# Wil-Lee/NN_BVH

Measured on AMD Instinct MI355X. Metric: Mray/s (closest-hit + any-hit), higher is better.
Workload: dtype f32; 1 GPU; crown, 1000x1400: one wavefront pass of 8 spp per step (8 spp per GPU-film) — primary, bounce-1 and bounce-2 closest-hit, shadow any-hit towards the light quads (batches pre-generated, hence independent: ONE launch; the dependent form is dependent_step), rays in --ray-order tile (a caller-side order the reference's integrator does not form: ray_order_probe), RecordShadowRayResult + RGBFilm::AddSam; sample_sets=4, geometry=procedural stand-in for crown (3548192 tris; data/crown.npz absent), tree=sah, triangles=3548192, nodes=7032259, rays_primary=11200000, rays_bounce=7410327, rays_bounce2=4392209, parallelism=tile-sharded x1, BVH replicated, film all-gather after the pass

## Files before the change

### nn_bvh_amd/build.py

```python
import concurrent.futures
import hashlib
import os
import shutil
import subprocess

HERE = os.path.dirname(os.path.abspath(__file__))
CSRC = os.path.join(HERE, "csrc")
LIB = os.path.join(HERE, "libnnbvh_hip.so")
SOURCES = ["bvh_trace.hip", "wavefront.hip", "wavefront2.hip", "wavefront_items.hip", "bvh_build_gpu.hip", "bvh_bake.hip", "interaction.hip", "film.hip", "kd_trace.hip", "kd_build_gpu.hip", "kd_bake.hip", "bvh_capi.cpp", "capi_two_level.cpp", "capi_trace.cpp", "capi_kd.cpp", "capi_wavefront.cpp", "capi_shading.cpp", "bvh_build.cpp", "kd_build.cpp"]
HEADERS = ["bvh_trace.h", "trace_instance.h", "top_table.h", "trace_math.h", "stream_access.h", "spawn_math.h", "anim_math.h", "alpha_texture_math.h", "wavefront2.h", "walk_math.h", "wavefront.h", "bvh_build_gpu.h", "interaction.h", "interaction_math.h", "wavefront_items.h", "kd_trace.h", "kd_build_gpu.h", "kd_device_util.h", "nnbvh_internal.h", "capi_internal.h", os.path.join("..", "..", "include", "nnbvh.h")]
CFLAGS = ["-O3", "--offload-arch=gfx950", "-ffp-contract=off", "-fPIC", "-std=c++17",
          "-Wall", "-Wno-unused-function", "-Wno-pass-failed"]
FLAGS = CFLAGS + ["-shared"]


def _hipcc():
    hipcc = shutil.which("hipcc") or "/opt/rocm/bin/hipcc"
    if not os.path.exists(hipcc):
        raise RuntimeError("hipcc not found: cannot build libnnbvh_hip.so")
    return hipcc


def _sources():
    return [s for s in SOURCES if os.path.exists(os.path.join(CSRC, s))]


def _deps_mtime():
    deps = [os.path.join(CSRC, f) for f in HEADERS] + [os.path.abspath(__file__)]
    return max(os.path.getmtime(d) for d in deps if os.path.exists(d))


def _stale():
    if not os.path.exists(LIB):
        return True
    t = os.path.getmtime(LIB)
    return _deps_mtime() > t or any(os.path.getmtime(os.path.join(CSRC, s)) > t for s in _sources())


def _build(out, extra=(), force=False, verbose=False, jobs=None):
    hipcc = _hipcc()
    tag = hashlib.sha1(" ".join(extra).encode()).hexdigest()[:10] if extra else "product"
    objdir = os.path.join(HERE, "_obj", tag)
    os.makedirs(objdir, exist_ok=True)
    hdr_t = _deps_mtime()
    todo, objs = [], []
    for s in _sources():
        src = os.path.join(CSRC, s)
        obj = os.path.join(objdir, s.rsplit(".", 1)[0] + ".o")
        objs.append(obj)
        if force or not os.path.exists(obj) or os.path.getmtime(obj) < max(hdr_t, os.path.getmtime(src)):
            todo.append([hipcc] + CFLAGS + list(extra) + ["-c", "-o", obj, src])

    def run(cmd):
        if verbose:
            print(" ".join(cmd), flush=True)
        subprocess.run(cmd, check=True, cwd=CSRC)

    jobs = jobs or min(len(todo) or 1, max(1, (os.cpu_count() or 2) - 1), 6)
    with concurrent.futures.ThreadPoolExecutor(jobs) as ex:
        list(ex.map(run, todo))
    run([hipcc, "--offload-arch=gfx950", "-shared", "-fPIC", "-o", out] + objs)
    return out


def build_stats(verbose=False):
    return _build(os.path.join(HERE, "libnnbvh_hip_stats.so"), ["-DNNBVH_STATS"], verbose=verbose)


def build_variant(name, defines, verbose=False, flags=()):
    return _build(os.path.join(HERE, f"libnnbvh_hip_{name}.so"), list(flags) + [f"-D{d}" for d in defines],
                  verbose=verbose)


def build(force=False, verbose=False):
    if not force and not _stale():
        return LIB
    return _build(LIB, force=force, verbose=verbose)


if __name__ == "__main__":
    import sys
    if len(sys.argv) > 1:
        print(build_variant(sys.argv[1], sys.argv[2:], verbose=True))
    else:
        print(build(force=True, verbose=True))
```

### nn_bvh_amd/csrc/bvh_capi.cpp

```cpp
#include <algorithm>
#include <cmath>
#include <cstring>
#include <limits>
#include <vector>

#include "alpha_texture_math.h"
#include "bvh_build_gpu.h"
#include "capi_internal.h"
#include "top_table.h"

namespace nnbvh {

static thread_local std::string g_error;
void set_error(const std::string &msg) { g_error = msg; }

}

using namespace nnbvh;

static bool validate_tree(const nnbvh_linear_node *nodes, int root, int n_tree, const nnbvh_prim *prims,
                          int n_prims, bool allow_instances, std::vector<uint8_t> &covered,
                          std::vector<uint8_t> &leaf_last, int *depth_out) {
    if (n_tree < 1) {
        set_error("scene_create: tree has no nodes");
        return false;
    }
    const int n_nodes = root + n_tree;
    struct Frame {
        int node, end, depth;
    };
    std::vector<Frame> st;
    st.push_back({root, n_nodes, 0});
    int visited = 0, max_depth = 0;
    while (!st.empty()) {
        Frame f = st.back();
        st.pop_back();
        ++visited;
        if (f.node < 0 || f.node >= f.end) {
            set_error("scene_create: node index outside its subtree range");
            return false;
        }
        max_depth = std::max(max_depth, f.depth);
        const nnbvh_linear_node &nd = nodes[f.node];
        for (int k = 0; k < 3; ++k)
            if (!(nd.pmin[k] <= nd.pmax[k])) {
                set_error("scene_create: node bounds with min > max (or NaN)");
                return false;
            }
        if (nd.nprims > 0) {
            if (f.node + 1 != f.end) {
                set_error("scene_create: leaf does not close its subtree range (not a DFS layout)");
                return false;
            }
            if (nd.offset < 0 || (int64_t)nd.offset + nd.nprims > n_prims) {
                set_error("scene_create: leaf primitive range out of bounds");
                return false;
            }
            for (int i = 0; i < nd.nprims; ++i) {
                if (covered[(size_t)nd.offset + i]) {
                    set_error("scene_create: primitive referenced by two leaves");
                    return false;
                }
                covered[(size_t)nd.offset + i] = 1;
                if (!allow_instances && prims[(size_t)nd.offset + i].kind == NNBVH_PRIM_INSTANCE) {
                    set_error("scene_create: nested instances are not supported");
                    return false;
                }
            }
            leaf_last[(size_t)nd.offset + nd.nprims - 1] = 1;
        } else {
            if (nd.axis > 2) {
                set_error("scene_create: interior node axis > 2");
                return false;
            }
            const int c0 = f.node + 1, c1 = nd.offset;
            if (c1 <= c0 || c1 >= f.end) {
                set_error("scene_create: secondChildOffset outside the node's subtree range");
                return false;
            }
            st.push_back({c1, f.end, f.depth + 1});
            st.push_back({c0, c1, f.depth + 1});
        }
    }
    if (visited != n_tree) {
        set_error("scene_create: unreachable nodes in the array");
        return false;
    }
    *depth_out = max_depth;
    return true;
}

// ... 683 lines not shown
    }
    std::memcpy(out, s->bounds, sizeof s->bounds);
    return NNBVH_OK;
}

int nnbvh_scene_info(const nnbvh_scene *s, int64_t out[6]) {
    if (!s || !out) {
        set_error("scene_info: null argument");
        return NNBVH_ERR_ARG;
    }
    out[0] = s->n_interior;
    out[1] = s->n_slots;
    out[2] = s->depth;
    out[3] = (int64_t)s->device_bytes;
    out[4] = grid_blocks(const_cast<nnbvh_scene *>(s), 0);
    out[5] = s->window;
    return NNBVH_OK;
}

int nnbvh_scene_read(const nnbvh_scene *s, int what, void *out, size_t bytes) {
    if (!s || !out) {
        set_error("scene_read: null argument");
        return NNBVH_ERR_ARG;
    }
    if (what < 0 || what > 4) {
        set_error("scene_read: unknown array (0 interior records, 1 primitive stream, 2 animation table, 3 alpha-texture "
                  "table, 4 alpha texel pool)");
        return NNBVH_ERR_ARG;
    }
    if (what >= 3) {
        if (!s->d_alpha_tex) {
            set_error("scene_read: the scene has no alpha textures");
            return NNBVH_ERR_ARG;
        }
        const void *from = what == 3 ? (const void *)s->d_alpha_tex : (const void *)s->d_alpha_texels;
        const size_t size = what == 3 ? (size_t)s->n_alpha_tex * 48 : (size_t)s->n_alpha_texels * 4;
        if (bytes != size) {
            set_error("scene_read: " + std::to_string(bytes) + " bytes asked for, the array has " + std::to_string(size));
            return NNBVH_ERR_ARG;
        }
        DeviceGuard guard(s->device);
        if (!guard.ok) return NNBVH_ERR_DEVICE;
        if (!hip_ok(hipDeviceSynchronize(), "scene_read") || !hip_ok(hipMemcpy(out, from, bytes, hipMemcpyDeviceToHost), "scene_read"))
            return NNBVH_ERR_DEVICE;
        return NNBVH_OK;
    }
    if (what == 2 && !s->d_anim) {
        set_error("scene_read: the scene has no animation table");
        return NNBVH_ERR_ARG;
    }
    const void *src = what == 0 ? (const void *)s->d_wide : what == 1 ? (const void *)s->d_prims : (const void *)s->d_anim;
    const size_t have = what == 0   ? (size_t)s->n_interior * sizeof(WideNode)
                        : what == 1 ? (size_t)s->n_slots * 16
                                    : (size_t)s->n_anim * kAnimStride * sizeof(float);
    if (bytes != have) {
        set_error("scene_read: " + std::to_string(bytes) + " bytes asked for, the array has " + std::to_string(have));
        return NNBVH_ERR_ARG;
    }
    if (bytes == 0) return NNBVH_OK;
    DeviceGuard guard(s->device);
    if (!guard.ok) return NNBVH_ERR_DEVICE;
    if (!hip_ok(hipDeviceSynchronize(), "scene_read") || !hip_ok(hipMemcpy(out, src, bytes, hipMemcpyDeviceToHost), "scene_read"))
        return NNBVH_ERR_DEVICE;
    return NNBVH_OK;
}

int nnbvh_scene_sched_stats(nnbvh_scene *s, uint64_t out[20], int reset) {
    if (!s || !out) {
        set_error("scene_sched_stats: null argument");
        return NNBVH_ERR_ARG;
    }
    std::memset(out, 0, nnbvh::kSchedStatWords * sizeof(uint64_t));
    if (!s->d_stats) return NNBVH_OK;
    DeviceGuard guard(s->device);
    if (!guard.ok) return NNBVH_ERR_DEVICE;
    if (!hip_ok(hipDeviceSynchronize(), "scene_sched_stats") ||
        !hip_ok(hipMemcpy(out, s->d_stats, nnbvh::kSchedStatWords * sizeof(uint64_t), hipMemcpyDeviceToHost),
                "scene_sched_stats"))
        return NNBVH_ERR_DEVICE;
    if (reset) (void)hipMemset(s->d_stats, 0, nnbvh::kSchedStatWords * sizeof(unsigned long long));
    return NNBVH_OK;
}

int nnbvh_scene_set_option(nnbvh_scene *s, const char *key, int value) {
    if (!s || !key) {
        set_error("set_option: null argument");
        return NNBVH_ERR_ARG;
    }
    std::lock_guard<std::mutex> lock(s->mu);
    std::string k(key);
    if (k == "stack_window") {
        if (value != 4 && value != 8 && value != 16) {
            set_error("set_option: stack_window must be 4, 8 or 16");
            return NNBVH_ERR_ARG;
        }
        s->window = value;
    } else if (k == "blocks_per_cu") {
        if (value < 0 || value > 8) {
            set_error("set_option: blocks_per_cu must be 0..8");
            return NNBVH_ERR_ARG;
        }
        s->blocks_per_cu = value;
    } else if (k == "int_repeat") {
        if (value < 1 || value > 16) {
            set_error("set_option: int_repeat must be 1..16");
            return NNBVH_ERR_ARG;
        }
        s->int_repeat = value;
    } else if (k == "host_chunk") {
        if (value < 1024) {
            set_error("set_option: host_chunk must be at least 1024 rays");
            return NNBVH_ERR_ARG;
        }
        s->host_chunk = value;
    } else if (k == "prim_repeat") {
        if (value < 1 || value > 16) {
            set_error("set_option: prim_repeat must be 1..16");
            return NNBVH_ERR_ARG;
        }
        s->prim_repeat = value;
    } else if (k == "fused_batches") {
        s->fused_batches = value ? 1 : 0;
    } else if (k == "top_table") {
        s->use_top = value ? 1 : 0;
    } else if (k == "top_burst") {
        if (value < 1 || value > 65) {
            set_error("set_option: top_burst must be 1..65");
            return NNBVH_ERR_ARG;
        }
        s->top_burst = value;
    } else if (k == "xcd_queues") {
        s->xcd_queues = value ? 1 : 0;
    } else if (k == "prim_weight") {
        if (value < 1 || value > 64) {
            set_error("set_option: prim_weight must be 1..64");
            return NNBVH_ERR_ARG;
        }
        s->prim_weight = value;
    } else if (k == "refill_weight") {
        if (value < 1 || value > 64) {
            set_error("set_option: refill_weight must be 1..64");
            return NNBVH_ERR_ARG;
        }
        s->refill_weight = value;
    } else {
        set_error("set_option: unknown key");
        return NNBVH_ERR_ARG;
    }
    return NNBVH_OK;
}

}

Workspace *nnbvh::workspace_for(nnbvh_scene *s, hipStream_t stream) {
    auto it = s->workspaces.find(stream);
    if (it != s->workspaces.end()) return &it->second;
    Workspace w;
    const size_t spill_bytes = (size_t)std::max(s->depth - 2, 1) * (size_t)s->max_grid_threads * sizeof(uint2);
    if (!hip_ok(hipMalloc((void **)&w.queue, kMaxFusedBatches * kMaxQueues * kQueueStrideWords * sizeof(unsigned)),
                "hipMalloc(queue)"))
        return nullptr;
    if (!hip_ok(hipMalloc((void **)&w.spill, spill_bytes), "hipMalloc(spill)")) {
        (void)hipFree(w.queue);
        return nullptr;
    }
    return &(s->workspaces[stream] = w);
// ... 2 lines not shown
```

### nn_bvh_amd/csrc/bvh_trace.h

```cpp
#pragma once
#include <hip/hip_runtime.h>
#include <stdint.h>

#include "../../include/nnbvh.h"
#include "nnbvh_internal.h"
#include "trace_instance.h"
#include "walk_math.h"

namespace nnbvh {

constexpr int kBlockThreads = 256;
constexpr int kMaxQueues = 8;
constexpr int kQueueStrideWords = 32;
constexpr int kMaxFusedBatches = 4;
constexpr int kSchedStatWords = 20;
constexpr int kFusedIndexBits = 28;

struct TraceParams {
    const float4 *wide;
    const float4 *prims;
    float rootMin[3], rootMax[3];
    int rootRef;
    const nnbvh_ray *rays;
    nnbvh_hit *hits;
    uint8_t *occluded;
    int32_t *visitedOut;
    int32_t *testsOut;
    long n;
    const int32_t *nDev;
    unsigned *queue;
    int nQueues;
    int primWeight;
    int refillWeight;
    int hasHostPrims;
    int intRepeat;
    int primRepeat;
    int fits32;
    unsigned long long *stats;
    uint2 *spill;
    const float *anim;
    int nBatches;
    unsigned anyMask;
    const nnbvh_ray *bRays[kMaxFusedBatches];
    void *bOut[kMaxFusedBatches];
    long bN[kMaxFusedBatches];
    const int32_t *bNDev[kMaxFusedBatches];
    nnbvh_ray_soa soa;
    nnbvh_ray_soa bSoa[kMaxFusedBatches];
    int hcCap;
    int32_t *hcCount;
    int32_t *hcBefore;
    int32_t *hcPrim;
    int32_t *hcInst;
    int bHcCap[kMaxFusedBatches];
    int32_t *bHcCount[kMaxFusedBatches];
    int32_t *bHcBefore[kMaxFusedBatches];
    int32_t *bHcPrim[kMaxFusedBatches];
    int32_t *bHcInst[kMaxFusedBatches];
    ShadingMeshDevice wMesh;
    WalkParams walk;
    const float4 *alphaTex;
    const float *alphaTexels;
    const float4 *top;
    int nTop;
    int topBurst;
};

hipError_t launch_zero_queue(unsigned *queue, int words, hipStream_t stream);
hipError_t launch_zero_words(int32_t *words, long n, int maxBlocks, hipStream_t stream);

hipError_t launch_trace(const TraceInstance &is, const TraceParams &p, int blocks, hipStream_t stream, int *occupancy);

}
```

### nn_bvh_amd/csrc/bvh_trace.hip

```cpp
#include <hip/hip_runtime.h>
#include <stdint.h>
#include <array>
#include <cstring>
#include <utility>

#include "bvh_trace.h"
#include "alpha_texture_math.h"
#include "anim_math.h"
#include "spawn_math.h"
#include "stream_access.h"
#include "trace_math.h"
#include "walk_math.h"

namespace nnbvh {

constexpr int kDone = (int)0x80000000;
constexpr int kReturn = (int)0x80000001;
constexpr int kEnter = (int)0x80000002;

#ifndef NNBVH_MINW_CLOSEST
#define NNBVH_MINW_CLOSEST 6
#endif
#ifndef NNBVH_MINW_ANY
#define NNBVH_MINW_ANY 6
#endif
#ifndef NNBVH_LEAN_EXTRA_WAVES
#define NNBVH_LEAN_EXTRA_WAVES 2
#endif
#ifndef NNBVH_MINW_ALPHA
#define NNBVH_MINW_ALPHA 5
#endif
#ifndef NNBVH_MINW_ALPHA_PATCH
#define NNBVH_MINW_ALPHA_PATCH 3
#endif
#ifndef NNBVH_MINW_ALPHA_TEX
#define NNBVH_MINW_ALPHA_TEX 4
#endif
#ifndef NNBVH_MINW_WALK_LEAN
#define NNBVH_MINW_WALK_LEAN 4
#endif
#ifndef NNBVH_MINW_WALK
#define NNBVH_MINW_WALK 4
#endif
constexpr int min_waves(int modew, int inst, int patch, int alpha) {
    if (inst) return 1;
    if (modew >= 4) return patch ? NNBVH_MINW_WALK : NNBVH_MINW_WALK_LEAN;
    if (alpha == 2) return NNBVH_MINW_ALPHA_PATCH;
    if (alpha == 3) return NNBVH_MINW_ALPHA_TEX;
    if (alpha) return NNBVH_MINW_ALPHA;
    return ((modew == 0 || modew == 3) ? NNBVH_MINW_CLOSEST : NNBVH_MINW_ANY) + (patch ? 0 : NNBVH_LEAN_EXTRA_WAVES);
}
#ifndef NNBVH_ANIM_ENTER_WEIGHT
#define NNBVH_ANIM_ENTER_WEIGHT 8
#endif
template <typename T>
__device__ __forceinline__ T pick_batch(const T (&a)[kMaxFusedBatches], int b) {
    static_assert(kMaxFusedBatches == 4, "written out for four batches");
    return b == 0 ? a[0] : (b == 1 ? a[1] : (b == 2 ? a[2] : a[3]));
}

#define BVH_BEGIN_RAY(R0, R1)                                                                                         \
    do {                                                                                                              \
        r.o = {(R0).x, (R0).y, (R0).z};                                                                               \
        tMax = (R0).w;                                                                                                \
        const V3 d = {(R1).x, (R1).y, (R1).z};                                                                        \
        if (PATCH) {                                                                                                  \
            cold[kColdD][lane] = d.x;                                                                                 \
            cold[kColdD + 1][lane] = d.y;                                                                             \
            cold[kColdD + 2][lane] = d.z;                                                                             \
        }                                                                                                             \
                                                                                          \
        r.inv = {1.0f / d.x, 1.0f / d.y, 1.0f / d.z};                                                                 \
        ray_shear(r, d);                                                                                              \
        if constexpr (kTop) {                                                                                         \
            hit0 = __int_as_float(-1);                                                                                \
            hit1 = hit2 = hit3 = 0.0f;                                                                                \
        } else if (MODE == 0 || MODE == 3) {                                                                          \
            cold[kColdHit][lane] = __int_as_float(-1);                                                                \
            cold[kColdHit + 1][lane] = 0.0f;                                                                          \
            cold[kColdHit + 2][lane] = 0.0f;                                                                          \
            cold[kColdHit + 3][lane] = 0.0f;                                                                          \
        }                                                                                                             \
        if (INST) {                                                                                                   \
            cold[kHitInst][lane] = 0.0f;                                                                              \
            cold[kCurInst][lane] = 0.0f;                                                                              \
            cold[kColdTime][lane] = (R1).w;                                 \
            floor = -1;                                                                                               \
        }                                                                                                             \
        if (!kLean && (HOSTC || p.hasHostPrims)) cold[kColdHost][lane] = 0.0f;           \
        if constexpr (WALK != 0) {                                                                                    \
            cold[kWalkD][lane] = (R1).x;                                                                              \
            cold[kWalkD + 1][lane] = (R1).y;                                                                          \
            cold[kWalkD + 2][lane] = (R1).z;                                                                          \
            cold[kWalkTime][lane] = (R1).w;                                                                           \
            cold[kWalkTMax][lane] = (R0).w;                                                                           \
        }                                                                                                             \
        visited = 1;                                                                                    \
        tests = 0;                                                                                                    \
        found = false;                                                                                                \
        sp = base = 0;                                                                                                \
        float tEntry;                                                                                                 \
        const bool rootHit = slab_partial(p.rootMin[0], p.rootMin[1], p.rootMin[2], p.rootMax[0], p.rootMax[1],       \
                                          p.rootMax[2], r, tEntry) &&                                                 \
                             (tEntry < tMax);                                                                         \
        cur = rootHit ? p.rootRef : kDone;                                                                            \
    } while (0)

template <int MODEW, int W, int INST, int PATCH, int ALPHA = 0, int SOA = 0, int HOSTC = 0>
__global__ __launch_bounds__(kBlockThreads, min_waves(MODEW, INST, PATCH, ALPHA))
void trace_kernel(TraceParams p) {
    constexpr int WALK = MODEW >= 4 ? MODEW - 3 : 0;
    constexpr int MODE = WALK ? 0 : MODEW;
    static_assert(!WALK || (MODEW <= 5 && W == 8 && INST != 2 && !ALPHA && !SOA && !HOSTC),
                  "walk instances: the plain record-reading closest-hit form at window 8");
    static_assert(PATCH || !INST, "two-level scenes need the ray direction");
    static_assert(PATCH || !ALPHA, "the alpha test hashes the ray direction");
    static_assert(ALPHA != 3 || (INST == 0 && W == 8 && MODE != 3), "textured alpha: flat scenes, window 8, modes 0 / 1 / 2");
    static_assert(!HOSTC || (PATCH && (MODE == 0 || MODE == 2 || (MODE == 3 && !ALPHA && W == 8)) && !SOA),
                  "candidate mode: general instances of modes 0 / 2 / 3");
    __shared__ float s_stack[kBlockThreads / 64][W][2][64];
    constexpr bool kLean = !PATCH && !INST;
    constexpr int kColdRi = 0, kColdD = 1, kColdHit = kLean ? 0 : (PATCH ? 4 : 1),
                  kColdHost = kColdHit + ((MODE == 0 || MODE == 3) ? 4 : 0);
    constexpr int kColdBase = kColdHost + (kLean ? 0 : 1);
    constexpr int kSaveO = kColdBase, kSaveInv = kColdBase + 3, kSaveShear = kColdBase + 6,
                  kSaveKz = kColdBase + 9, kSaveTmax = kColdBase + 10, kSaveD = kColdBase + 11,
                  kResume = kColdBase + 14, kCurInst = kColdBase + 15, kHitInst = kColdBase + 16,
                  kInnerHit = kColdBase + 17, kColdTime = kColdBase + 18, kPendSlot = kColdBase + 19;
    constexpr int kColdWalk = kColdBase + (INST ? 20 : 0);
    [[maybe_unused]] constexpr int kWalkD = kColdWalk, kWalkTime = kColdWalk + 3, kWalkTMax = kColdWalk + 4,
                                   kWalkCalls = kColdWalk + 5;
    constexpr int kColdFields = kColdWalk + (WALK ? 6 : 0);
    constexpr bool kTop = kLean && MODEW == 3;

    const int lane = threadIdx.x & 63;
    const int wave = threadIdx.x >> 6;
    const int gtid = blockIdx.x * kBlockThreads + threadIdx.x;
    float(*stk)[2][64] = s_stack[wave];
    float(*cold)[64] = nullptr;
    [[maybe_unused]] const float4 *top = nullptr;
    if constexpr (kTop) {
        __shared__ float4 s_top[kTopRecords * 4];
        static_assert(kTopRecords * 4 <= kBlockThreads, "one float4 per thread copies the table");
        if ((int)threadIdx.x < p.nTop * 4) s_top[threadIdx.x] = p.top[threadIdx.x];
        __syncthreads();
        top = s_top;
    } else {
        __shared__ float s_cold[kBlockThreads / 64][kColdFields > 0 ? kColdFields : 1][64];
        cold = s_cold[wave];
    }
    [[maybe_unused]] float hit0 = 0.0f, hit1 = 0.0f, hit2 = 0.0f, hit3 = 0.0f;
    int riReg = -1;
    if (!kLean) cold[kColdRi][lane] = __int_as_float(-1);
    const long spillStride = (long)gridDim.x * kBlockThreads;

    int q = 0;
    if (p.nQueues > 1) {
        unsigned xcc;
        asm volatile("s_getreg_b32 %0, hwreg(HW_REG_XCC_ID)" : "=s"(xcc));
        q = (int)(xcc & 0xf) % p.nQueues;
    }
    int queuesTried = 0;
    int curBatch = 0;
    long nRays = p.n;
    if (p.nDev) {
        const long nd = (long)*p.nDev;
        nRays = nd < 0 ? 0 : (nd < nRays ? nd : nRays);
    }

#ifdef NNBVH_STATS
    unsigned long long st[kSchedStatWords] = {0, 0, 0, 0, 0, 0, 0, 0, 0, 0, 0, 0, 0, 0, 0, 0, 0, 0, 0, 0};
    unsigned long long stPrev = __builtin_amdgcn_s_memtime();
    int stKind = 2;
#endif
    RayState r;
    RayMasks masks = {0ull, 0ull, 0ull, 0ull, 0ull, 0ull};
    float tMax = 0.0f;
    int visited = 0, tests = 0;
    int cur = kDone, sp = 0, base = 0;
    int floor = -1;
    bool found = false;
    bool exhausted = false;
    [[maybe_unused]] int topBurst = 65;
    if constexpr (kTop) {
        topBurst = p.topBurst;
        asm volatile("" : "+s"(topBurst));
    }

    auto pop_entry = [&](int &ref, float &key) {
        --sp;
        ref = __float_as_int(stk[sp & (W - 1)][0][lane]);
        key = stk[sp & (W - 1)][1][lane];
        asm volatile("" : "+v"(ref), "+v"(key));
        if (sp < base) {
            const uint2 e = p.spill[(long)sp * spillStride + gtid];
            base = sp;
            ref = (int)e.x;
            key = __uint_as_float(e.y);
            asm volatile("" : "+v"(ref), "+v"(key));
        }
        if (MODE != 2) visited += 1;
    };
    auto pop_next = [&]() -> int {
        const int lowest = (INST && floor > 0) ? floor : 0;
        const int none = (INST && floor >= 0) ? kReturn : kDone;
        if (sp <= lowest) return none;
        int ref;
        float key;
        pop_entry(ref, key);
        if (key < tMax) return ref;
        while (sp > lowest) {
            pop_entry(ref, key);
            if (key < tMax) return ref;
        }
        return none;
    };

    auto enter_instance = [&](int slot, unsigned flags, float4 s0, float4 s1, float4 s2) {
        const float4 s3 = p.prims[slot + 3], s4 = p.prims[slot + 4], s5 = p.prims[slot + 5];
        const V3 dOuter = {cold[kColdD][lane], cold[kColdD + 1][lane], cold[kColdD + 2][lane]};
        cold[kSaveO][lane] = r.o.x;
        cold[kSaveO + 1][lane] = r.o.y;
        cold[kSaveO + 2][lane] = r.o.z;
        cold[kSaveInv][lane] = r.inv.x;
        cold[kSaveInv + 1][lane] = r.inv.y;
        cold[kSaveInv + 2][lane] = r.inv.z;
        cold[kSaveShear][lane] = r.sx;
        cold[kSaveShear + 1][lane] = r.sy;
        cold[kSaveShear + 2][lane] = r.sz;
        cold[kSaveKz][lane] = __int_as_float(r.kz);
        cold[kSaveTmax][lane] = tMax;
        cold[kSaveD][lane] = dOuter.x;
        cold[kSaveD + 1][lane] = dOuter.y;
        cold[kSaveD + 2][lane] = dOuter.z;
        cold[kResume][lane] = __int_as_float((flags & kPrimLast) ? kDone : ~(slot + 6));
        cold[kCurInst][lane] = __int_as_float(__float_as_int(s0.w) + 1);
        cold[kInnerHit][lane] = 0.0f;
// ... 163 lines not shown
                } else {
                    hit = patch_test(r, rd, tMax, {s0.x, s0.y, s0.z}, {s1.x, s1.y, s1.z},
                                     {s2.x, s2.y, s2.z}, {s3.x, s3.y, s3.z}, x0, x1, th);
                }
            }
            bool closestLane = MODE == 0;
            if (MODE == 3 && hit)
                closestLane = !((p.anyMask >> ((kLean ? riReg : __float_as_int(cold[kColdRi][lane])) >> kFusedIndexBits)) & 1u);
            if (hit) {
                if (closestLane) {
                    if constexpr (kTop) {
                        hit0 = s0.w;
                        hit1 = x0;
                        hit2 = x1;
                        hit3 = x2;
                    } else {
                        cold[kColdHit][lane] = s0.w;
                        cold[kColdHit + 1][lane] = x0;
                        cold[kColdHit + 2][lane] = x1;
                        cold[kColdHit + 3][lane] = x2;
                    }
                    tMax = th;
                    if (INST) {
                        cold[kHitInst][lane] = cold[kCurInst][lane];
                        cold[kInnerHit][lane] = 1.0f;
                    }
                    if constexpr (HOSTC && MODE == 0) {
                        const int c = __float_as_int(cold[kColdHost][lane]);
                        if (c > 0) p.hcBefore[__float_as_int(cold[kColdRi][lane])] = c;
                    }
                    if constexpr (HOSTC && MODE == 3) {
                        const int c = __float_as_int(cold[kColdHost][lane]);
                        if (c > 0) {
                            const int tag = __float_as_int(cold[kColdRi][lane]);
                            pick_batch(p.bHcBefore, tag >> kFusedIndexBits)[tag & ((1 << kFusedIndexBits) - 1)] = c;
                        }
                    }
                } else {
                    found = true;
                }
            }
            if (MODE != 0 && found) cur = kDone;
            else if (flags & kPrimLast) cur = pop_next();
            else cur = ~next;
        }
    };

    auto interior_math = [&](const float4 q0, const float4 q1, const float4 q2, const float4 q3) {
        const int ref0 = __float_as_int(q3.x), ref1 = __float_as_int(q3.y);
        const int axis = __float_as_int(q3.z);
        const bool swap = ((r.kz >> axis) & 1) != 0;
        const float k0 = kLean ? slab_entry_key(q0.x, q0.y, q0.z, q0.w, q1.x, q1.y, r, masks)
                               : slab_entry_key(q0.x, q0.y, q0.z, q0.w, q1.x, q1.y, r);
        const float k1 = kLean ? slab_entry_key(q1.z, q1.w, q2.x, q2.y, q2.z, q2.w, r, masks)
                               : slab_entry_key(q1.z, q1.w, q2.x, q2.y, q2.z, q2.w, r);
        const int nearRef = swap ? ref1 : ref0, farRef = swap ? ref0 : ref1;
        const float nearT = swap ? k1 : k0, farT = swap ? k0 : k1;
        visited += 1;
        const bool doPush = (MODE == 1) || (farT < __builtin_inff());
        if (doPush && sp - base == W - 1) {
            uint2 e;
            e.x = __float_as_uint(stk[base & (W - 1)][0][lane]);
            e.y = __float_as_uint(stk[base & (W - 1)][1][lane]);
            p.spill[(long)base * spillStride + gtid] = e;
            ++base;
        }
        stk[sp & (W - 1)][0][lane] = __int_as_float(farRef);
        stk[sp & (W - 1)][1][lane] = farT;
        sp += doPush ? 1 : 0;
        if (MODE == 0 || MODE == 3) visited += doPush ? 0 : 1;
        cur = nearT < tMax ? nearRef : pop_next();
    };
    auto interior_step = [&]() {
#ifdef NNBVH_STATS
        st[14] += 1;
        st[15] += __popcll(__ballot(cur >= 0));
        if (kTop) st[13] += __popcll(__ballot(cur >= 0 && (cur & kTopTag) != 0));
#endif
        if constexpr (kTop) {
            if (cur >= 0) {
                typedef float v4f __attribute__((ext_vector_type(4)));
                const unsigned at = (unsigned)cur << 6;
                v4f q0, q1, q2, q3;
                if (cur & kTopTag) {
                    const v4f *rec = reinterpret_cast<const v4f *>(reinterpret_cast<const char *>(top) + at);
                    q3 = rec[3];
                    q0 = rec[0], q1 = rec[1], q2 = rec[2];
                    asm volatile("" : "+v"(q0), "+v"(q1), "+v"(q2), "+v"(q3));
                } else {
                    const v4f *rec = reinterpret_cast<const v4f *>(reinterpret_cast<const char *>(p.wide) + at);
                    q3 = rec[3];
                    q0 = rec[0], q1 = rec[1], q2 = rec[2];
                }
                interior_math({q0.x, q0.y, q0.z, q0.w}, {q1.x, q1.y, q1.z, q1.w}, {q2.x, q2.y, q2.z, q2.w},
                              {q3.x, q3.y, q3.z, q3.w});
            }
        } else if (cur >= 0) {
            const float4 *rec = kLean ? reinterpret_cast<const float4 *>(reinterpret_cast<const char *>(p.wide) + ((unsigned)cur << 6))
                                      : p.wide + 4 * (long)cur;
            const float4 q3 = rec[3];
            const float4 q0 = rec[0], q1 = rec[1], q2 = rec[2];
            interior_math(q0, q1, q2, q3);
        }
    };
    [[maybe_unused]] auto table_step = [&]() {
        if (((unsigned)cur >> 30) == 1u) {
            typedef float v4f __attribute__((ext_vector_type(4)));
            const v4f *rec = reinterpret_cast<const v4f *>(reinterpret_cast<const char *>(top) + ((unsigned)cur << 6));
            const v4f q3 = rec[3];
            const v4f q0 = rec[0], q1 = rec[1], q2 = rec[2];
            interior_math({q0.x, q0.y, q0.z, q0.w}, {q1.x, q1.y, q1.z, q1.w}, {q2.x, q2.y, q2.z, q2.w},
                          {q3.x, q3.y, q3.z, q3.w});
        }
    };

    for (;;) {
#ifdef NNBVH_STATS
        {
            const unsigned long long now = __builtin_amdgcn_s_memtime();
            st[10 + stKind] += now - stPrev;
            stPrev = now;
        }
#endif
        const bool isInt = cur >= 0;
        const bool isIdle = cur == kDone;
        const int nInt = __popcll(__ballot(isInt));
        const unsigned long long idleMask = __ballot(isIdle);
        const int nIdle = __popcll(idleMask);
        const int nEnter = (INST == 2 && NNBVH_ANIM_ENTER_WEIGHT > 0) ? __popcll(__ballot(cur == kEnter)) : 0;
        const int nPrim = 64 - nInt - nIdle - nEnter;

        const int sI = nInt * 16, sP = nPrim * p.primWeight;
        const int sR = exhausted ? 0 : nIdle * p.refillWeight;
#ifdef NNBVH_STATS
        unsigned long long &stTrips = (nIdle == 64 || (sR > sI && sR > sP)) ? st[4]
                                      : ((sP > sI || nInt == 0) ? st[2] : st[0]);
        (&stTrips)[0] += 1;
        (&stTrips)[1] += (nIdle == 64 || (sR > sI && sR > sP)) ? nIdle
                         : ((sP > sI || nInt == 0) ? nPrim : nInt);
        stKind = (&stTrips == &st[4]) ? 2 : ((&stTrips == &st[2]) ? 1 : 0);
        if (&stTrips == &st[0]) {
            st[6] += nInt;
            st[7] += nPrim;
            st[8] += nIdle;
        }
#endif
        if (nIdle == 64 || (sR > sI && sR > sP)) {
            const int ri = isIdle ? (kLean ? riReg : __float_as_int(cold[kColdRi][lane])) : -1;
            [[maybe_unused]] bool goOn = false, capped = false;
            [[maybe_unused]] V3 nextO = {0.0f, 0.0f, 0.0f}, nextD = {0.0f, 0.0f, 0.0f};
            [[maybe_unused]] float nextTMax = 1.0f, nextTime = 0.0f;
            if constexpr (WALK != 0) {
                if (ri >= 0) {
                    const float4 r0 = {r.o.x, r.o.y, r.o.z, cold[kWalkTMax][lane]};
                    const float4 r1 = {cold[kWalkD][lane], cold[kWalkD + 1][lane], cold[kWalkD + 2][lane],
                                       cold[kWalkTime][lane]};
                    const float4 h0 = {cold[kColdHit][lane], tMax, cold[kColdHit + 1][lane], cold[kColdHit + 2][lane]};
                    float4 h1 = {cold[kColdHit + 3][lane], __int_as_float(visited), __int_as_float(tests),
                                 INST ? cold[kHitInst][lane] : 0.0f};
                    if (!kLean && p.hasHostPrims && cold[kColdHost][lane] != 0.0f) h1.w = __int_as_float(-1);
                    const ShadingMeshDevice &sm = p.wMesh;
                    const MeshView wm = {sm.verts, sm.triVerts, sm.patchVerts, sm.normals, sm.uvs, sm.tangents,
                                         sm.faceIndices, sm.triFlags, sm.nTris, sm.defaultFlags, sm.instances,
                                         sm.nInstances, sm.anim, sm.animFwd};
                    if constexpr (WALK == 1) {
                        goOn = w2_str_item<PATCH != 0>(wm, r0, r1, h0, h1, ri, p.walk.primClass, p.walk.nPrimClass,
                                                       p.walk.pLight, p.walk.state, nextO, nextD);
                        nextTMax = r0.w;
                        nextTime = r1.w;
                        if (goOn && nextD.x == 0.0f && nextD.y == 0.0f && nextD.z == 0.0f) goOn = false;
                    } else {
                        goOn = w2_or_item<PATCH != 0>(wm, r0, r1, h0, h1, ri, p.walk.p1, p.walk.material,
                                                      p.walk.primMaterial, p.walk.nPrimMaterial, p.walk.st,
                                                      p.walk.selHits, p.walk.selRays, nextO, nextD);
                    }
                    if (goOn) {
// ... 224 lines not shown
                if constexpr (kTop) {
#ifdef NNBVH_STATS
                    unsigned long long stT0 = 0;
                    bool stTable = false;
#endif
                    for (;;) {
                        const int nTag = __popcll(__ballot(((unsigned)cur >> 30) == 1u));
                        if (nTag < topBurst) break;
#ifdef NNBVH_STATS
                        if (!stTable) stT0 = __builtin_amdgcn_s_memtime();
                        stTable = true;
                        st[16] += 1;
                        st[17] += nTag;
#endif
                        table_step();
                    }
#ifdef NNBVH_STATS
                    if (stTable) {
                        const unsigned long long stT1 = __builtin_amdgcn_s_memtime();
                        st[18] += stT1 - stT0;
                        stPrev += stT1 - stT0;
                    }
#endif
                }
                interior_step();
                if (p.intRepeat > 1 && __ballot(cur >= 0) != 0ull) {
                    interior_step();
                    if (p.intRepeat > 2 && __ballot(cur >= 0) != 0ull) {
                        interior_step();
                        for (int rep = 3; rep < p.intRepeat && __ballot(cur >= 0) != 0ull; ++rep) interior_step();
                    }
                }
            } else {
            int rep = 0;
            do {
                interior_step();
            } while (++rep < p.intRepeat && __ballot(cur >= 0) != 0ull);
            }
        }
    }
#ifdef NNBVH_STATS
    if (lane == 0 && p.stats)
        for (int k = 0; k < kSchedStatWords; ++k) atomicAdd(&p.stats[k], st[k]);
#endif
}
#undef BVH_BEGIN_RAY

__global__ void zero_queue_kernel(unsigned *queue, int words) {
    for (int i = threadIdx.x; i < words; i += blockDim.x) queue[i] = 0u;
}
hipError_t launch_zero_queue(unsigned *queue, int words, hipStream_t stream) {
    hipLaunchKernelGGL(zero_queue_kernel, dim3(1), dim3(256), 0, stream, queue, words);
    return hipGetLastError();
}

__global__ void zero_words_kernel(int32_t *words, long n) {
    for (long i = (long)blockIdx.x * blockDim.x + threadIdx.x; i < n; i += (long)gridDim.x * blockDim.x) words[i] = 0;
}
hipError_t launch_zero_words(int32_t *words, long n, int maxBlocks, hipStream_t stream) {
    long blocks = (n + 255) / 256;
    blocks = blocks < 1 ? 1 : (blocks < maxBlocks ? blocks : maxBlocks);
    hipLaunchKernelGGL(zero_words_kernel, dim3((unsigned)blocks), dim3(256), 0, stream, words, n);
    return hipGetLastError();
}

struct TraceEntry {
    TraceInstance is;
    void (*kernel)(TraceParams);
};
template <size_t I>
constexpr TraceEntry trace_entry() {
    constexpr TraceInstance t = kTraceInstances[I];
    return {t, trace_kernel<t.mode, t.window, t.inst, t.patch, t.alpha, t.soa, t.hostc>};
}
template <size_t... I>
constexpr std::array<TraceEntry, sizeof...(I)> trace_table(std::index_sequence<I...>) {
    return {{trace_entry<I>()...}};
}
static const auto kTraceTable = trace_table(std::make_index_sequence<std::size(kTraceInstances)>());

hipError_t launch_trace(const TraceInstance &is, const TraceParams &p, int blocks, hipStream_t stream, int *occupancy) {
    for (const TraceEntry &e : kTraceTable) {
        if (std::memcmp(&e.is, &is, sizeof is) != 0) continue;
        if (occupancy) return hipOccupancyMaxActiveBlocksPerMultiprocessor(occupancy, e.kernel, kBlockThreads, 0);
        hipLaunchKernelGGL(e.kernel, dim3((unsigned)blocks), dim3(kBlockThreads), 0, stream, p);
        return hipGetLastError();
    }
    return hipErrorInvalidValue;
}

}
```

### nn_bvh_amd/csrc/capi_trace.cpp

```cpp
#include <algorithm>
#include <cstring>
#include <thread>

#include "capi_internal.h"

using namespace nnbvh;

int nnbvh::grid_blocks(nnbvh_scene *s, int mode, int candidates) {
    int per_cu = s->blocks_per_cu;
    if (per_cu <= 0) {
        TraceInstance is{};
        if (!pick_trace_instance(scene_traits(s), mode, candidates > 0, false, &is) ||
            launch_trace(is, TraceParams{}, 0, nullptr, &per_cu) != hipSuccess || per_cu <= 0)
            per_cu = std::max(1, std::min(8, 160 / (s->window * 2)));
    }
    per_cu = std::min(per_cu, 8);
    return s->n_cus * per_cu;
}

bool nnbvh::zero_candidates(int n_cus, const nnbvh_host_candidates *hc, int64_t n, bool closest, hipStream_t stream) {
    return hip_ok(launch_zero_words(hc->count, (long)n, n_cus * 8, stream), "candidate count reset launch") &&
           (!closest || !hc->before ||
            hip_ok(launch_zero_words(hc->before, (long)n, n_cus * 8, stream), "candidate before reset launch"));
}

static TraceParams scene_params(const nnbvh_scene *s, const Workspace *w) {
    TraceParams p{};
    p.wide = s->d_wide;
    p.prims = s->d_prims;
    std::memcpy(p.rootMin, s->bounds, 12);
    std::memcpy(p.rootMax, s->bounds + 3, 12);
    p.rootRef = s->root_ref;
    p.queue = w->queue;
    p.nQueues = s->xcd_queues ? kMaxQueues : 1;
    p.primWeight = s->prim_weight;
    p.refillWeight = s->refill_weight;
    p.stats = s->d_stats;
    p.intRepeat = s->int_repeat;
    p.topBurst = s->top_burst;
    p.primRepeat = s->prim_repeat;
    p.fits32 = scene_fits32(s);
    p.hasHostPrims = s->has_host_prims;
    p.spill = w->spill;
    p.anim = s->d_anim;
    p.alphaTex = (const float4 *)s->d_alpha_tex;
    p.alphaTexels = s->d_alpha_texels;
    return p;
}

static int run_instance(bool have, const TraceInstance &is, const TraceParams &p, int blocks, int queue_words,
                        hipStream_t stream, const char *what) {
    if (!hip_ok(launch_zero_queue(p.queue, queue_words, stream), "queue reset launch")) return NNBVH_ERR_DEVICE;
    const int64_t need = (p.n + kBlockThreads - 1) / kBlockThreads;
    if (need < blocks) blocks = (int)std::max<int64_t>(need, 1);
    const hipError_t e = have ? launch_trace(is, p, blocks, stream, nullptr) : hipErrorInvalidValue;
    return hip_ok(e, what) ? NNBVH_OK : NNBVH_ERR_DEVICE;
}

static int run_trace(nnbvh_scene *s, hipStream_t stream, int mode, bool candidates, bool soa, const TraceParams &p,
                     int queue_words, const char *what) {
    TraceInstance is{};
    const bool have = pick_trace_instance(scene_traits(s), mode, candidates, soa, &is);
    return run_instance(have, is, p, grid_blocks(s, mode, candidates), queue_words, stream, what);
}

int nnbvh::launch(nnbvh_scene *s, Workspace *w, hipStream_t stream, const TraceJob &job) {
    TraceParams p = scene_params(s, w);
    if (job.soa) p.soa = *job.soa;
    p.rays = (const nnbvh_ray *)job.rays;
    p.hits = (nnbvh_hit *)job.hits;
    p.occluded = (uint8_t *)job.occluded;
    p.visitedOut = (int32_t *)job.visited;
    p.testsOut = (int32_t *)job.tests;
    p.n = (long)job.n;
    p.nDev = job.d_n;
    if (const nnbvh_host_candidates *hc = job.hc) {
        int32_t *before = job.mode == 0 ? hc->before : nullptr;
        const size_t bytes = (size_t)job.n * sizeof(int32_t);
        if (!job.hc_zeroed &&
            (!hip_ok(hipMemsetAsync(hc->count, 0, bytes, stream), "hipMemsetAsync(count)") ||
             (before && !hip_ok(hipMemsetAsync(before, 0, bytes, stream), "hipMemsetAsync(before)"))))
            return NNBVH_ERR_DEVICE;
        if (s->has_host_prims) {
            p.hcCap = hc->capacity;
            p.hcCount = hc->count;
            p.hcBefore = before;
            p.hcPrim = hc->prim;
            p.hcInst = hc->instance;
        }
    }
    const bool candidates = job.hc && s->has_host_prims && job.hc->capacity > 0;
    return run_trace(s, stream, job.mode, candidates, !job.rays, p, kMaxQueues * kQueueStrideWords,
                     "trace kernel launch");
}

const char *nnbvh::walk_refusal(const nnbvh_scene *s) {
    if (s->instanced && s->d_anim)
        return "the scene holds AnimatedPrimitive instances (the INST = 2 kernels), which have no walk instances";
    if (s->has_alpha)
        return "the scene holds alpha-tested primitives on the device (the ALPHA kernels), which have no walk instances";
    return nullptr;
}

int nnbvh::launch_walk(nnbvh_scene *s, Workspace *w, hipStream_t stream, const WalkJob &k) {
    TraceParams p = scene_params(s, w);
    p.rays = (const nnbvh_ray *)k.rays;
    p.n = (long)k.n;
    p.nDev = k.d_n;
    p.wMesh = *k.mesh;
    p.walk = k.a;
    TraceInstance is{};
    int form = 0;
    const ShadingMeshDevice &m = *k.mesh;
    if (!pick_walk_instance(scene_traits(s), k.kind, m.patchVerts != nullptr, m.instances != nullptr, &is, &form))
        return run_instance(false, is, p, 0, kMaxQueues * kQueueStrideWords, stream, "walk kernel launch");
    int &per_cu = s->walk_blocks_per_cu[3 * (k.kind - 1) + form];
    if (per_cu == 0) {
        int occ = 0;
        per_cu = (launch_trace(is, p, 0, nullptr, &occ) == hipSuccess && occ > 0) ? std::min(occ, 8) : 2;
    }
    return run_instance(true, is, p, s->n_cus * per_cu, kMaxQueues * kQueueStrideWords, stream, "walk kernel launch");
}

int nnbvh::launch_fused_batches(nnbvh_scene *s, Workspace *w, hipStream_t stream, const nnbvh_batch *batches,
                                int n_batches, const int32_t *const *d_n, const nnbvh_ray_soa *const *soas,
                                const nnbvh_host_candidates *cands) {
    TraceParams p = scene_params(s, w);
    int64_t total = 0;
    bool candidates = false, soa = false;
    for (int i = 0; i < n_batches; ++i) {
        if (batches[i].n == 0) continue;
        const int b = p.nBatches++;
        p.bRays[b] = (const nnbvh_ray *)batches[i].d_rays;
        soa = soa || !batches[i].d_rays;
        p.bOut[b] = batches[i].d_out;
        p.bN[b] = (long)batches[i].n;
// ... 413 lines not shown
```

Baseline: 4934 Mray/s.

## Grow LDS top-of-tree table per block and use 1024-thread blocks for any-hit

```diff
diff --git a/nn_bvh_amd/build.py b/nn_bvh_amd/build.py
--- a/nn_bvh_amd/build.py
+++ b/nn_bvh_amd/build.py
@@ -8,7 +8,7 @@
 CSRC = os.path.join(HERE, "csrc")
 LIB = os.path.join(HERE, "libnnbvh_hip.so")
 SOURCES = ["bvh_trace.hip", "wavefront.hip", "wavefront2.hip", "wavefront_items.hip", "bvh_build_gpu.hip", "bvh_bake.hip", "interaction.hip", "film.hip", "kd_trace.hip", "kd_build_gpu.hip", "kd_bake.hip", "bvh_capi.cpp", "capi_two_level.cpp", "capi_trace.cpp", "capi_kd.cpp", "capi_wavefront.cpp", "capi_shading.cpp", "bvh_build.cpp", "kd_build.cpp"]
-HEADERS = ["bvh_trace.h", "trace_instance.h", "top_table.h", "trace_math.h", "stream_access.h", "spawn_math.h", "anim_math.h", "alpha_texture_math.h", "wavefront2.h", "walk_math.h", "wavefront.h", "bvh_build_gpu.h", "interaction.h", "interaction_math.h", "wavefront_items.h", "kd_trace.h", "kd_build_gpu.h", "kd_device_util.h", "nnbvh_internal.h", "capi_internal.h", os.path.join("..", "..", "include", "nnbvh.h")]
+HEADERS = ["bvh_trace.h", "trace_instance.h", "top_table.h", "top_extend.h", "trace_math.h", "stream_access.h", "spawn_math.h", "anim_math.h", "alpha_texture_math.h", "wavefront2.h", "walk_math.h", "wavefront.h", "bvh_build_gpu.h", "interaction.h", "interaction_math.h", "wavefront_items.h", "kd_trace.h", "kd_build_gpu.h", "kd_device_util.h", "nnbvh_internal.h", "capi_internal.h", os.path.join("..", "..", "include", "nnbvh.h")]
 CFLAGS = ["-O3", "--offload-arch=gfx950", "-ffp-contract=off", "-fPIC", "-std=c++17",
           "-Wall", "-Wno-unused-function", "-Wno-pass-failed"]
 FLAGS = CFLAGS + ["-shared"]
diff --git a/nn_bvh_amd/csrc/bvh_capi.cpp b/nn_bvh_amd/csrc/bvh_capi.cpp
--- a/nn_bvh_amd/csrc/bvh_capi.cpp
+++ b/nn_bvh_amd/csrc/bvh_capi.cpp
@@ -7,6 +7,7 @@
 #include "alpha_texture_math.h"
 #include "bvh_build_gpu.h"
 #include "capi_internal.h"
+#include "top_extend.h"
 #include "top_table.h"
 
 namespace nnbvh {
@@ -856,6 +857,46 @@
     return NNBVH_OK;
 }
 
+int nnbvh_debug_top_table(nnbvh_scene *s, int blocks, void *device_tables, int32_t *device_counts, void *host_table,
+                          int32_t *host_count, int32_t *capacity) {
+    if (!s || blocks < 1 || blocks > 4096 || !device_tables || !device_counts || !host_table || !host_count || !capacity) {
+        set_error("debug_top_table: bad argument");
+        return NNBVH_ERR_ARG;
+    }
+    const int cap = top_debug_capacity();
+    *capacity = cap;
+    DeviceGuard guard(s->device);
+    if (!guard.ok) return NNBVH_ERR_DEVICE;
+    std::vector<WideNode> table((size_t)s->n_top);
+    std::vector<int32_t> order;
+    if (s->n_top > 0 && !hip_ok(hipMemcpy(table.data(), s->d_top, table.size() * sizeof(WideNode), hipMemcpyDeviceToHost),
+                                "hipMemcpy(top table)"))
+        return NNBVH_ERR_DEVICE;
+    const auto fetch = [&](int32_t record, WideNode *out) {
+        if (record < 0 || record >= s->n_interior) return false;
+        return hip_ok(hipMemcpy(out, s->d_wide + 4 * (size_t)record, sizeof(WideNode), hipMemcpyDeviceToHost),
+                      "hipMemcpy(top record)");
+    };
+    if (!extend_top_table(fetch, cap, &table, &order)) return NNBVH_ERR_DEVICE;
+    *host_count = (int32_t)table.size();
+    std::memcpy(host_table, table.data(), table.size() * sizeof(WideNode));
+    const size_t bytes = (size_t)blocks * (size_t)cap * sizeof(WideNode);
+    float4 *d_out = nullptr;
+    int *d_n = nullptr;
+    bool ok = hip_ok(hipMalloc((void **)&d_out, bytes), "hipMalloc(debug tables)") &&
+              hip_ok(hipMalloc((void **)&d_n, (size_t)blocks * sizeof(int)), "hipMalloc(debug counts)") &&
+              hip_ok(hipMemset(d_out, 0, bytes), "hipMemset(debug tables)") &&
+              hip_ok(launch_top_table_debug(s->d_top, s->n_top, s->d_wide, blocks, d_out, d_n, nullptr),
+                     "top table debug launch") &&
+              hip_ok(hipDeviceSynchronize(), "top table debug kernel") &&
+              hip_ok(hipMemcpy(device_tables, d_out, bytes, hipMemcpyDeviceToHost), "hipMemcpy(debug tables)") &&
+              hip_ok(hipMemcpy(device_counts, d_n, (size_t)blocks * sizeof(int), hipMemcpyDeviceToHost),
+                     "hipMemcpy(debug counts)");
+    if (d_out) (void)hipFree(d_out);
+    if (d_n) (void)hipFree(d_n);
+    return ok ? NNBVH_OK : NNBVH_ERR_DEVICE;
+}
+
 int nnbvh_scene_set_option(nnbvh_scene *s, const char *key, int value) {
     if (!s || !key) {
         set_error("set_option: null argument");
diff --git a/nn_bvh_amd/csrc/bvh_trace.h b/nn_bvh_amd/csrc/bvh_trace.h
--- a/nn_bvh_amd/csrc/bvh_trace.h
+++ b/nn_bvh_amd/csrc/bvh_trace.h
@@ -69,6 +69,12 @@
 hipError_t launch_zero_queue(unsigned *queue, int words, hipStream_t stream);
 hipError_t launch_zero_words(int32_t *words, long n, int maxBlocks, hipStream_t stream);
 
+int trace_block_threads(const TraceInstance &is);
+
 hipError_t launch_trace(const TraceInstance &is, const TraceParams &p, int blocks, hipStream_t stream, int *occupancy);
 
+int top_debug_capacity();
+hipError_t launch_top_table_debug(const float4 *top, int nTop, const float4 *wide, int blocks, float4 *out, int *nOut,
+                                  hipStream_t stream);
+
 }
diff --git a/nn_bvh_amd/csrc/bvh_trace.hip b/nn_bvh_amd/csrc/bvh_trace.hip
--- a/nn_bvh_amd/csrc/bvh_trace.hip
+++ b/nn_bvh_amd/csrc/bvh_trace.hip
@@ -9,6 +9,7 @@
 #include "anim_math.h"
 #include "spawn_math.h"
 #include "stream_access.h"
+#include "top_extend.h"
 #include "trace_math.h"
 #include "walk_math.h"
 
@@ -50,6 +51,72 @@
     if (alpha) return NNBVH_MINW_ALPHA;
     return ((modew == 0 || modew == 3) ? NNBVH_MINW_CLOSEST : NNBVH_MINW_ANY) + (patch ? 0 : NNBVH_LEAN_EXTRA_WAVES);
 }
+#ifndef NNBVH_TOP_BLOCK
+#define NNBVH_TOP_BLOCK 1024
+#endif
+constexpr int block_threads(int modew, int inst, int patch) {
+    return (modew == 3 && !inst && !patch) ? NNBVH_TOP_BLOCK : kBlockThreads;
+}
+int trace_block_threads(const TraceInstance &is) { return block_threads(is.mode, is.inst, is.patch); }
+
+template <int BT>
+__device__ __forceinline__ int load_top_table(float4 *s_top, const float4 *top, int nTop, const float4 *wide) {
+    constexpr int kCap = top_lds_records(BT);
+    static_assert(kCap >= kTopRecords && kTopRecords * 4 <= BT, "one float4 per thread copies the scene's table");
+    static_assert(2 * kCap <= BT, "one (slot, child) pair per thread in a generation");
+    const int t = threadIdx.x, lane = t & 63, wave = t >> 6;
+    if (t < nTop * 4) s_top[t] = top[t];
+    __syncthreads();
+    int next = nTop;
+    if constexpr (kCap > kTopRecords) {
+        float *words = reinterpret_cast<float *>(s_top);
+        int begin = 0;
+        while (next < kCap && begin < next) {
+            const int end = next, nPairs = 2 * (end - begin), nGroups = (nPairs + 63) >> 6;
+            TopGroupScan scan;
+            int ref = -1;
+            for (int g = 0; g < nGroups; ++g) {
+                const int pair = 64 * g + lane;
+                int r = -1;
+                if (pair < nPairs) r = __float_as_int(words[(begin + (pair >> 1)) * 16 + 12 + (pair & 1)]);
+                scan.add(g, wave, __ballot(top_is_candidate(r)));
+                ref = g == wave ? r : ref;
+            }
+            const int slot = top_is_candidate(ref) ? scan.slot(lane, next, kCap) : -1;
+            __syncthreads();
+            if (slot >= 0) {
+                const float4 *rec = wide + 4 * (long)ref;
+                const float4 q0 = rec[0], q1 = rec[1], q2 = rec[2], q3 = rec[3];
+                s_top[4 * slot] = q0;
+                s_top[4 * slot + 1] = q1;
+                s_top[4 * slot + 2] = q2;
+                s_top[4 * slot + 3] = q3;
+                words[(begin + (t >> 1)) * 16 + 12 + (t & 1)] = __int_as_float(kTopTag | slot);
+            }
+            __syncthreads();
+            begin = end;
+            next = next + scan.total < kCap ? next + scan.total : kCap;
+        }
+    }
+    return next;
+}
+template <int BT>
+__global__ __launch_bounds__(BT) void top_table_debug_kernel(const float4 *top, int nTop, const float4 *wide,
+                                                             float4 *out, int *nOut) {
+    constexpr int kCap = top_lds_records(BT);
+    __shared__ float4 s_top[kCap * 4];
+    const int n = load_top_table<BT>(s_top, top, nTop, wide);
+    for (int k = threadIdx.x; k < n * 4; k += BT) out[(long)blockIdx.x * kCap * 4 + k] = s_top[k];
+    if (threadIdx.x == 0) nOut[blockIdx.x] = n;
+}
+int top_debug_capacity() { return top_lds_records(NNBVH_TOP_BLOCK); }
+hipError_t launch_top_table_debug(const float4 *top, int nTop, const float4 *wide, int blocks, float4 *out, int *nOut,
+                                  hipStream_t stream) {
+    hipLaunchKernelGGL(top_table_debug_kernel<NNBVH_TOP_BLOCK>, dim3((unsigned)blocks), dim3(NNBVH_TOP_BLOCK), 0,
+                       stream, top, nTop, wide, out, nOut);
+    return hipGetLastError();
+}
+
 #ifndef NNBVH_ANIM_ENTER_WEIGHT
 #define NNBVH_ANIM_ENTER_WEIGHT 8
 #endif
@@ -107,7 +174,7 @@
     } while (0)
 
 template <int MODEW, int W, int INST, int PATCH, int ALPHA = 0, int SOA = 0, int HOSTC = 0>
-__global__ __launch_bounds__(kBlockThreads, min_waves(MODEW, INST, PATCH, ALPHA))
+__global__ __launch_bounds__(block_threads(MODEW, INST, PATCH), min_waves(MODEW, INST, PATCH, ALPHA))
 void trace_kernel(TraceParams p) {
     constexpr int WALK = MODEW >= 4 ? MODEW - 3 : 0;
     constexpr int MODE = WALK ? 0 : MODEW;
@@ -118,7 +185,8 @@
     static_assert(ALPHA != 3 || (INST == 0 && W == 8 && MODE != 3), "textured alpha: flat scenes, window 8, modes 0 / 1 / 2");
     static_assert(!HOSTC || (PATCH && (MODE == 0 || MODE == 2 || (MODE == 3 && !ALPHA && W == 8)) && !SOA),
                   "candidate mode: general instances of modes 0 / 2 / 3");
-    __shared__ float s_stack[kBlockThreads / 64][W][2][64];
+    constexpr int BT = block_threads(MODEW, INST, PATCH);
+    __shared__ float s_stack[BT / 64][W][2][64];
     constexpr bool kLean = !PATCH && !INST;
     constexpr int kColdRi = 0, kColdD = 1, kColdHit = kLean ? 0 : (PATCH ? 4 : 1),
                   kColdHost = kColdHit + ((MODE == 0 || MODE == 3) ? 4 : 0);
@@ -135,24 +203,22 @@
 
     const int lane = threadIdx.x & 63;
     const int wave = threadIdx.x >> 6;
-    const int gtid = blockIdx.x * kBlockThreads + threadIdx.x;
+    const int gtid = blockIdx.x * BT + threadIdx.x;
     float(*stk)[2][64] = s_stack[wave];
     float(*cold)[64] = nullptr;
     [[maybe_unused]] const float4 *top = nullptr;
     if constexpr (kTop) {
-        __shared__ float4 s_top[kTopRecords * 4];
-        static_assert(kTopRecords * 4 <= kBlockThreads, "one float4 per thread copies the table");
-        if ((int)threadIdx.x < p.nTop * 4) s_top[threadIdx.x] = p.top[threadIdx.x];
-        __syncthreads();
+        __shared__ __attribute__((aligned(1024))) float4 s_top[top_lds_records(BT) * 4];
+        load_top_table<BT>(s_top, p.top, p.nTop, p.wide);
         top = s_top;
     } else {
-        __shared__ float s_cold[kBlockThreads / 64][kColdFields > 0 ? kColdFields : 1][64];
+        __shared__ float s_cold[BT / 64][kColdFields > 0 ? kColdFields : 1][64];
         cold = s_cold[wave];
     }
     [[maybe_unused]] float hit0 = 0.0f, hit1 = 0.0f, hit2 = 0.0f, hit3 = 0.0f;
     int riReg = -1;
     if (!kLean) cold[kColdRi][lane] = __int_as_float(-1);
-    const long spillStride = (long)gridDim.x * kBlockThreads;
+    const long spillStride = (long)gridDim.x * BT;
 
     int q = 0;
     if (p.nQueues > 1) {
@@ -482,16 +548,30 @@
                 typedef float v4f __attribute__((ext_vector_type(4)));
                 const unsigned at = (unsigned)cur << 6;
                 v4f q0, q1, q2, q3;
-                if (cur & kTopTag) {
-                    const v4f *rec = reinterpret_cast<const v4f *>(reinterpret_cast<const char *>(top) + at);
-                    q3 = rec[3];
-                    q0 = rec[0], q1 = rec[1], q2 = rec[2];
-                    asm volatile("" : "+v"(q0), "+v"(q1), "+v"(q2), "+v"(q3));
-                } else {
-                    const v4f *rec = reinterpret_cast<const v4f *>(reinterpret_cast<const char *>(p.wide) + at);
-                    q3 = rec[3];
-                    q0 = rec[0], q1 = rec[1], q2 = rec[2];
-                }
+                const unsigned long long tagged = __ballot((cur & kTopTag) != 0);
+                const unsigned ldsAt = at + (unsigned)reinterpret_cast<uintptr_t>(top);
+                unsigned long long active;
+                asm volatile(
+                    "s_mov_b64 %[act], exec\n\t"
+                    "s_andn2_b64 exec, exec, %[tag]\n\t"
+                    "s_cbranch_execz 1f\n\t"
+                    "global_load_dwordx4 %[q3], %[at], %[wide] offset:48\n\t"
+                    "global_load_dwordx4 %[q0], %[at], %[wide]\n\t"
+                    "global_load_dwordx4 %[q1], %[at], %[wide] offset:16\n\t"
+                    "global_load_dwordx4 %[q2], %[at], %[wide] offset:32\n"
+                    "1:\n\t"
+                    "s_and_b64 exec, %[act], %[tag]\n\t"
+                    "s_cbranch_execz 2f\n\t"
+                    "ds_read_b128 %[q3], %[lds] offset:48\n\t"
+                    "ds_read_b128 %[q0], %[lds]\n\t"
+                    "ds_read_b128 %[q1], %[lds] offset:16\n\t"
+                    "ds_read_b128 %[q2], %[lds] offset:32\n"
+                    "2:\n\t"
+                    "s_mov_b64 exec, %[act]\n\t"
+                    "s_waitcnt vmcnt(0) lgkmcnt(0)"
+                    : [q0] "=&v"(q0), [q1] "=&v"(q1), [q2] "=&v"(q2), [q3] "=&v"(q3), [act] "=&s"(active)
+                    : [at] "v"(at), [lds] "v"(ldsAt), [wide] "s"(p.wide), [tag] "s"(tagged)
+                    : "scc");
                 interior_math({q0.x, q0.y, q0.z, q0.w}, {q1.x, q1.y, q1.z, q1.w}, {q2.x, q2.y, q2.z, q2.w},
                               {q3.x, q3.y, q3.z, q3.w});
             }
@@ -882,8 +962,9 @@
 hipError_t launch_trace(const TraceInstance &is, const TraceParams &p, int blocks, hipStream_t stream, int *occupancy) {
     for (const TraceEntry &e : kTraceTable) {
         if (std::memcmp(&e.is, &is, sizeof is) != 0) continue;
-        if (occupancy) return hipOccupancyMaxActiveBlocksPerMultiprocessor(occupancy, e.kernel, kBlockThreads, 0);
-        hipLaunchKernelGGL(e.kernel, dim3((unsigned)blocks), dim3(kBlockThreads), 0, stream, p);
+        const int threads = trace_block_threads(is);
+        if (occupancy) return hipOccupancyMaxActiveBlocksPerMultiprocessor(occupancy, e.kernel, threads, 0);
+        hipLaunchKernelGGL(e.kernel, dim3((unsigned)blocks), dim3(threads), 0, stream, p);
         return hipGetLastError();
     }
     return hipErrorInvalidValue;
diff --git a/nn_bvh_amd/csrc/capi_trace.cpp b/nn_bvh_amd/csrc/capi_trace.cpp
--- a/nn_bvh_amd/csrc/capi_trace.cpp
+++ b/nn_bvh_amd/csrc/capi_trace.cpp
@@ -13,6 +13,8 @@
         if (!pick_trace_instance(scene_traits(s), mode, candidates > 0, false, &is) ||
             launch_trace(is, TraceParams{}, 0, nullptr, &per_cu) != hipSuccess || per_cu <= 0)
             per_cu = std::max(1, std::min(8, 160 / (s->window * 2)));
+        else
+            per_cu *= trace_block_threads(is) / kBlockThreads;
     }
     per_cu = std::min(per_cu, 8);
     return s->n_cus * per_cu;
@@ -51,7 +53,9 @@
 static int run_instance(bool have, const TraceInstance &is, const TraceParams &p, int blocks, int queue_words,
                         hipStream_t stream, const char *what) {
     if (!hip_ok(launch_zero_queue(p.queue, queue_words, stream), "queue reset launch")) return NNBVH_ERR_DEVICE;
-    const int64_t need = (p.n + kBlockThreads - 1) / kBlockThreads;
+    const int threads = have ? trace_block_threads(is) : kBlockThreads;
+    blocks = std::max(1, (int)((int64_t)blocks * kBlockThreads / threads));
+    const int64_t need = (p.n + threads - 1) / threads;
     if (need < blocks) blocks = (int)std::max<int64_t>(need, 1);
     const hipError_t e = have ? launch_trace(is, p, blocks, stream, nullptr) : hipErrorInvalidValue;
     return hip_ok(e, what) ? NNBVH_OK : NNBVH_ERR_DEVICE;
diff --git a/nn_bvh_amd/csrc/top_extend.h b/nn_bvh_amd/csrc/top_extend.h
--- /dev/null
+++ b/nn_bvh_amd/csrc/top_extend.h
@@ -0,0 +1,68 @@
+#pragma once
+#include <algorithm>
+#include <cstdint>
+#include <vector>
+
+#include "nnbvh_internal.h"
+
+namespace nnbvh {
+
+constexpr int top_lds_records(int block_threads) { return block_threads / 4 - 1; }
+
+NNBVH_HD inline bool top_is_candidate(int32_t ref) { return ref >= 0 && (ref & kTopTag) == 0; }
+
+NNBVH_HD inline int top_popcount(unsigned long long m) { return __builtin_popcountll(m); }
+
+struct TopGroupScan {
+    int before = 0, total = 0;
+    unsigned long long own = 0ull;
+    NNBVH_HD void add(int g, int mine, unsigned long long mask) {
+        const int n = top_popcount(mask);
+        before += g < mine ? n : 0;
+        own = g == mine ? mask : own;
+        total += n;
+    }
+    NNBVH_HD int slot(int bit, int next, int capacity) const {
+        const int s = next + before + top_popcount(own & ((1ull << bit) - 1ull));
+        return s < capacity ? s : -1;
+    }
+};
+
+template <class Fetch>
+bool extend_top_table(Fetch fetch, int capacity, std::vector<WideNode> *table, std::vector<int32_t> *order) {
+    int begin = 0, next = (int)table->size();
+    while (next < capacity && begin < next) {
+        const int end = next, n_pairs = 2 * (end - begin), n_groups = (n_pairs + 63) >> 6;
+        const auto ref_of = [&](int pair) -> int32_t & {
+            WideNode &w = (*table)[(size_t)(begin + (pair >> 1))];
+            return (pair & 1) ? w.ref1 : w.ref0;
+        };
+        std::vector<unsigned long long> masks((size_t)n_groups, 0ull);
+        for (int pair = 0; pair < n_pairs; ++pair)
+            if (top_is_candidate(ref_of(pair))) masks[(size_t)(pair >> 6)] |= 1ull << (pair & 63);
+        int total = 0;
+        table->resize((size_t)std::min(capacity, next + n_pairs));
+        for (int mine = 0; mine < n_groups; ++mine) {
+            TopGroupScan scan;
+            for (int g = 0; g < n_groups; ++g) scan.add(g, mine, masks[(size_t)g]);
+            total = scan.total;
+            for (int bit = 0; bit < 64; ++bit) {
+                if (!((masks[(size_t)mine] >> bit) & 1ull)) continue;
+                const int slot = scan.slot(bit, next, capacity);
+                if (slot < 0) continue;
+                int32_t &ref = ref_of(64 * mine + bit);
+                WideNode w;
+                if (!fetch(ref, &w)) return false;
+                (*table)[(size_t)slot] = w;
+                order->push_back(ref);
+                ref = kTopTag | slot;
+            }
+        }
+        begin = end;
+        next = std::min(capacity, next + total);
+        table->resize((size_t)next);
+    }
+    return true;
+}
+
+}
```

New measurement: 5045 Mray/s, median of 6. 1.02x the previous value.
